# acerbilab/gpyreg

Measured on AMD Instinct MI355X. Metric: GP-fits/sec (NLL+grad, N=4096 D=10), higher is better.
Workload: dtype f64

## Files before the change

### gpyreg_amd/_lib.py

```python

from __future__ import annotations

import ctypes as C
import os
import threading

import numpy as np

_HERE = os.path.dirname(os.path.abspath(__file__))
LIB_PATH = os.environ.get("GPYREG_AMD_LIB") or os.path.join(_HERE, "lib", "libgpcore.so")

K_SE, K_MATERN, K_RQ, K_SE_ISO, K_MATERN_ISO = range(5)
F64, F32 = 0, 1
KLO_ZERO, KLO_ROW, KLO_COL = 0, 1, 2
KHI_FULL, KHI_ROW, KHI_COL = 0, 1, 2

_dp = C.c_void_p
_ip = C.c_void_p
_vp = C.c_void_p
_dpp = C.POINTER(C.c_double)

SIGNATURES = {
    "gpc_create": (C.c_int, [C.c_int, C.POINTER(_vp)]),
    "gpc_destroy": (None, [_vp]),
# ... 331 lines not shown
        self._check(self._lib.gpc_set_option(self._h, name.encode(), int(value)), "gpc_set_option")

    @_serial
    def get_option(self, name: str) -> int:
        v = C.c_int()
        self._check(self._lib.gpc_get_option(self._h, name.encode(), C.byref(v)), "gpc_get_option")
        return v.value

    @_serial
    def last_lauum_timing(self):
        a, b = C.c_double(), C.c_double()
        self._lib.gpc_last_lauum_timing(self._h, C.byref(a), C.byref(b))
        return a.value, b.value

    @_serial
    def mfma_peak(self, dtype=F64):
        t, cyc, ghz = C.c_double(), C.c_double(), C.c_double()
        rc = self._lib.gpc_mfma_peak(self._h, dtype, C.byref(t), C.byref(cyc), C.byref(ghz))
        self._check(rc, "gpc_mfma_peak")
        return t.value, cyc.value, ghz.value

    @_serial
    def debug_gemm(self, A, B, Cm, M, N, K, a_kmajor, b_kmajor, alpha=1.0, beta=0, klo=0, khi=0,
                   lower_only=False, dtype=F64, force_bt=0):
        A, B = _f64(A), _f64(B)
        Cm = _f64(Cm).copy()
        flags = int(bool(lower_only)) | {0: 0, 64: 0x100, 128: 0x200, 12864: 0x400}[force_bt]
        rc = self._lib.gpc_debug_gemm(self._h, dtype, M, N, K, int(a_kmajor), int(b_kmajor),
                                      float(alpha), int(beta), klo, khi, flags, _ptr(A),
                                      _ptr(B), _ptr(Cm))
        self._check(rc, "gpc_debug_gemm")
        return Cm

    @_serial
    def debug_factor(self, A, want_inv=True, dtype=F64):
        A = _f64(A)
        n = A.shape[0]
        L, W = np.empty((n, n)), np.empty((n, n))
        Ainv = np.empty((n, n)) if want_inv else None
        logdet = C.c_double()
        info = C.c_int()
        rc = self._lib.gpc_debug_factor(self._h, dtype, n, _ptr(A), _ptr(L), _ptr(W), _ptr(Ainv),
                                        C.byref(logdet), C.byref(info))
        self._check(rc, "gpc_debug_factor")
        return L, W, Ainv, logdet.value, info.value

    @_serial
    def debug_cov(self, which, kid, degree, hyp_cov, X, dtype=F64, kscale=1.0, sl=1.0, dvec=None, X_star=None,
                  mat=None, vec=None):
        code = {"build": 0, "front": 1, "cross": 2, "trace": 3}[which]
# ... 340 lines not shown
```

### gpyreg_amd/csrc/common.h

```cpp
#pragma once
#include <hip/hip_runtime.h>

#include <cmath>
#include <cstdint>
#include <cstdio>
#include <cstring>
#include <string>
#include <vector>

namespace gpc {

constexpr int TILE = 128;
constexpr int WAVE = 64;

inline int pad_tile(int n) { return ((n + TILE - 1) / TILE) * TILE; }

inline int chunk_from_budget(int S, size_t per, size_t shared, size_t budget, bool clamp_to_one) {
  if (budget < shared + per) return clamp_to_one ? 1 : 0;
  const size_t fit = (budget - shared) / per;
  return (int)(fit < (size_t)S ? fit : (size_t)S);
}

constexpr int LEAF_TIMEOUT = 1 << 30;

template <typename T>
struct MM;

template <>
struct MM<double> {
  using acc_t = double __attribute__((ext_vector_type(4)));
// ... 50 lines not shown
__device__ __forceinline__ bool cu_reserve_bail(const unsigned short* __restrict__ tbl, int* __restrict__ ctr) {
  __shared__ int bail_sh;
  if (threadIdx.x == 0) {
    unsigned hw, xcc;
    asm volatile("s_getreg_b32 %0, hwreg(HW_REG_HW_ID)" : "=s"(hw));
    asm volatile("s_getreg_b32 %0, hwreg(HW_REG_XCC_ID)" : "=s"(xcc));
    const unsigned cu = (hw >> 8) & 0xf, se = (hw >> 13) & 0x7;
    int bail = (tbl[(xcc & 7) * 8 + se] >> cu) & 1;
    if (!bail) {
      __hip_atomic_fetch_add(ctr + CTR_SURVIVORS, 1, __ATOMIC_RELAXED, __HIP_MEMORY_SCOPE_AGENT);
      __hip_atomic_fetch_add(ctr + CTR_STARTED, 1, __ATOMIC_RELEASE, __HIP_MEMORY_SCOPE_AGENT);
    } else {
      const int before = __hip_atomic_fetch_add(ctr + CTR_STARTED, 1, __ATOMIC_ACQ_REL, __HIP_MEMORY_SCOPE_AGENT);
      if (before == (int)gridDim.x - 1 &&
          __hip_atomic_load(ctr + CTR_SURVIVORS, __ATOMIC_ACQUIRE, __HIP_MEMORY_SCOPE_AGENT) == 0)
        bail = 0;
    }
    bail_sh = bail;
  }
  __syncthreads();
  return bail_sh != 0;
}

}
```

### gpyreg_amd/csrc/gemm.h

```cpp
#pragma once
#include "common.h"

#include <type_traits>

namespace gpc {

template <typename T>
constexpr int BKT_v = sizeof(T) == 4 ? 32 : 16;
template <typename T>
constexpr bool MM_SWZ = sizeof(T) == 4;
template <typename T>
constexpr int LDQ_v = MM_SWZ<T> ? BKT_v<T> : BKT_v<T> + 1;
constexpr int ldp_of(int BT) { return BT + 16; }
template <typename T>
constexpr int opsz_of(int BT) {
  return BKT_v<T> * (BT + 16) > BT * LDQ_v<T> ? BKT_v<T> * (BT + 16) : BT * LDQ_v<T>;
}

enum { KLO_ZERO = 0, KLO_ROW = 1, KLO_COL = 2 };
enum { KHI_FULL = 0, KHI_ROW = 1, KHI_COL = 2 };

struct GemmArgs {
  const void* A;
  const void* B;
  void* C;
  long long sA, sB, sC;
  int lda, ldb, ldc;
  int M, N, K;
  double alpha;
  int beta;
  int klo, khi, lower_only;
  int tiles_m, tiles_n;
  int flags = 0;
  const unsigned short* rsv = nullptr;
  int* ctr = nullptr;
  int ntiles = 0, batch = 0;
  double* colsq = nullptr;
  const double* ep_w = nullptr;
  long long ep_sw = 0;
  const double* ep_alpha = nullptr;
};
inline int g_gemm_flags = 8 | 16;

template <typename T, bool KM, int BT, int NT>
__device__ __forceinline__ unsigned stage_toff(int ld, int t) {
  constexpr int VEC = MM<T>::VEC;
  if constexpr (!KM) {
    constexpr int TPR = BKT_v<T> / VEC;
    return (unsigned)(t / TPR) * (unsigned)ld + (unsigned)((t % TPR) * VEC);
  } else {
    constexpr int VPR = BT / VEC;
    return (unsigned)(t / VPR) * (unsigned)ld + (unsigned)((t % VPR) * VEC);
  }
}
template <typename T, bool KM, int BT, int NT>
// ... 62 lines not shown
      return s[(r0 + l15) * LDQ_v<T> + (((k / VEC) ^ ((l15 >> 1) & 7)) * VEC) + (k % VEC)];
    } else {
      return s[(r0 + (lane & 15)) * LDQ_v<T> + kk + (lane >> 4)];
    }
  }
  else
    return s[(kk + (lane >> 4)) * ldp_of(BT) + r0 + (lane & 15)];
}

__device__ __forceinline__ void tri_tile(int tile, int& ti, int& tj) {
  int i = (int)((sqrtf(8.f * (float)tile + 1.f) - 1.f) * 0.5f);
  while (i * (i + 1) / 2 > tile) --i;
  while ((i + 1) * (i + 2) / 2 <= tile) ++i;
  ti = i;
  tj = tile - i * (i + 1) / 2;
}

#ifdef GPC_TILE_TRACE
__device__ unsigned long long g_tile_trace[2][4];
#define TILE_TS(k) do { if (HO && threadIdx.x == 0) { const long long _n = wall_clock64(); atomicAdd(&g_tile_trace[BT == 64][k], (unsigned long long)(_n - _ts)); _ts = _n; } } while (0)
#else
#define TILE_TS(k) do { } while (0)
#endif
template <typename T, bool AKM, bool BKM, int BT, int NW, int HO = 0, int EPI = 0, int BTN = BT>
__device__ __forceinline__ void gemm_tile(const GemmArgs& g, const int bx, const int by, T* __restrict__ smem) {
#ifdef GPC_TILE_TRACE
  long long _ts = wall_clock64();
  if (HO && threadIdx.x == 0) atomicAdd(&g_tile_trace[BT == 64][3], 1ull);
#endif
  using acc_t = typename MM<T>::acc_t;
  using vec_t = typename MM<T>::vec_t;
  constexpr int NT = 64 * NW;
  constexpr int NVA = (BT * BKT_v<T>) / (NT * MM<T>::VEC), NVB = (BTN * BKT_v<T>) / (NT * MM<T>::VEC);
  constexpr int OPSZA = opsz_of<T>(BT), OPSZB = opsz_of<T>(BTN), STG = OPSZA + OPSZB;
  constexpr int WCOLS = NW / 2;
  constexpr int WTM = BT / 2;
  constexpr int WTN = BTN / WCOLS;
  constexpr int MRM = WTM / 16, MRN = WTN / 16;
  static_assert(NVA >= 1 && NVB >= 1 && MRM >= 1 && MRN >= 1, "tile shape");
  const int t = threadIdx.x;
  const int lane = t & 63, w = t >> 6, wr = w / WCOLS, wc = w % WCOLS;

  int ti, tj;
  if (g.lower_only) {
    if constexpr (BTN == BT) {
      tri_tile(bx, ti, tj);
    } else {
      static_assert(BT == 2 * BTN, "lower tiles of a rectangular launch: two tile columns per tile row");
      int i = (int)((sqrtf(4.f * (float)bx + 1.f) - 1.f) * 0.5f);
      while (i * (i + 1) > bx) --i;
      while ((i + 1) * (i + 2) <= bx) ++i;
      ti = i;
      tj = bx - i * (i + 1);
    }
  } else if (g.khi == KHI_COL) {
    tj = g.tiles_n - 1 - bx / g.tiles_m;
    ti = bx % g.tiles_m;
  } else if (g.klo == KLO_COL) {
    tj = bx / g.tiles_m;
    ti = bx % g.tiles_m;
  } else if (g.khi == KHI_ROW) {
    ti = g.tiles_m - 1 - bx / g.tiles_n;
    tj = bx % g.tiles_n;
  } else {
    ti = bx / g.tiles_n;
    tj = bx % g.tiles_n;
  }
  const int m0 = ti * BT, n0 = tj * BTN;
  const int m128 = (m0 / TILE) * TILE, n128 = (n0 / TILE) * TILE;
  int k0 = g.klo == KLO_ROW ? m128 : (g.klo == KLO_COL ? n128 : 0);
  int k1 = g.khi == KHI_ROW ? m128 + TILE : (g.khi == KHI_COL ? n128 + TILE : g.K);
  if (k1 > g.K) k1 = g.K;
  const int nk = (k1 - k0) / BKT_v<T>;

  const T* __restrict__ A = reinterpret_cast<const T*>(g.A) + (size_t)by * g.sA;
  const T* __restrict__ B = reinterpret_cast<const T*>(g.B) + (size_t)by * g.sB;
  T* __restrict__ C = reinterpret_cast<T*>(g.C) + (size_t)by * g.sC;

  acc_t acc[MRM][MRN];
#pragma unroll
  for (int i = 0; i < MRM; ++i)
#pragma unroll
    for (int j = 0; j < MRN; ++j) acc[i][j] = acc_t{0, 0, 0, 0};
  constexpr bool TWO_LEVEL = sizeof(T) == 4;
  acc_t acc2[TWO_LEVEL ? MRM : 1][TWO_LEVEL ? MRN : 1];
  if constexpr (TWO_LEVEL) {
#pragma unroll
    for (int i = 0; i < MRM; ++i)
#pragma unroll
      for (int j = 0; j < MRN; ++j) acc2[i][j] = acc_t{0, 0, 0, 0};
  }

  if (nk > 0) {
    vec_t ra[NVA], rb[NVB];
    const unsigned toa = stage_toff<T, AKM, BT, NT>(g.lda, t) * (unsigned)sizeof(T),
                   tob = stage_toff<T, BKM, BTN, NT>(g.ldb, t) * (unsigned)sizeof(T);
// ... 12 lines not shown
        ua += (unsigned)(BKT_v<T> * sizeof(T));
      }
      if constexpr (BKM) {
        pb += rowsb;
        rsb = make_rsrc(pb);
      } else {
        ub += (unsigned)(BKT_v<T> * sizeof(T));
      }
    };
    constexpr int AUX = HO == 1 ? 16 : 0;
    g2r<T, AKM, BT, NT, AUX>(ra, rsa, ua, psa, toa);
    g2r<T, BKM, BTN, NT, AUX>(rb, rsb, ub, psb, tob);
    r2s<T, AKM, BT, NT>(smem, ra, t);
    r2s<T, BKM, BTN, NT>(smem + OPSZA, rb, t);
    next_slab();
    g2r<T, AKM, BT, NT, AUX>(ra, rsa, ua, psa, toa);
    g2r<T, BKM, BTN, NT, AUX>(rb, rsb, ub, psb, tob);
    __syncthreads();
    TILE_TS(0);

    T af[2][MRM], bf[2][MRN];
    auto load_frags = [&](int set, const T* a_s, const T* b_s, int kk) {
#pragma unroll
      for (int i = 0; i < MRM; ++i) af[set][i] = frag<T, AKM, BT>(a_s, wr * WTM + i * 16, kk, lane);
#pragma unroll
      for (int j = 0; j < MRN; ++j) bf[set][j] = frag<T, BKM, BTN>(b_s, wc * WTN + j * 16, kk, lane);
    };
    auto mfmas = [&](int set) {
#pragma unroll
      for (int i = 0; i < MRM; ++i)
#pragma unroll
        for (int j = 0; j < MRN; ++j) acc[i][j] = MM<T>::mma(af[set][i], bf[set][j], acc[i][j]);
    };
    constexpr int NMEM = NVA + NVB;
    constexpr int PER = (MRM * MRN) / NMEM;
    constexpr int REM = MRM * MRN - PER * NMEM;
    static_assert(PER >= 1, "interleave pattern");
    constexpr int KS = BKT_v<T> / 4;
    static_assert(KS >= 4 && KS % 2 == 0, "fragment sets alternate per k-step and wrap per slab");
    auto slab = [&](auto cur_c, auto wr_c, auto ld_c) {
      constexpr int CUR = decltype(cur_c)::value;
      constexpr bool WR = decltype(wr_c)::value, LD = decltype(ld_c)::value;
      const T* a_s = smem + CUR * STG;
      const T* b_s = a_s + OPSZA;
      T* a_n = smem + (CUR ^ 1) * STG;
#pragma unroll
      for (int ks = 0; ks < KS - 2; ++ks) {
        load_frags((ks + 1) & 1, a_s, b_s, 4 * (ks + 1));
        mfmas(ks & 1);
        __builtin_amdgcn_sched_group_barrier(0x100, MRM + MRN, 0);
        __builtin_amdgcn_sched_group_barrier(0x008, MRM * MRN, 0);
      }
      load_frags(1, a_s, b_s, 4 * (KS - 1));
      mfmas(0);
      if constexpr (WR) {
        r2s<T, AKM, BT, NT>(a_n, ra, t);
        r2s<T, BKM, BTN, NT>(a_n + OPSZA, rb, t);
      }
      __builtin_amdgcn_sched_group_barrier(0x100, MRM + MRN, 0);
#pragma unroll
      for (int q = 0; q < NMEM; ++q) {
        __builtin_amdgcn_sched_group_barrier(0x008, PER, 0);
        if constexpr (WR) __builtin_amdgcn_sched_group_barrier(0x200, 1, 0);
      }
      if constexpr (REM > 0) __builtin_amdgcn_sched_group_barrier(0x008, REM, 0);
      __syncthreads();
      if constexpr (LD) {
        next_slab();
        g2r<T, AKM, BT, NT, AUX>(ra, rsa, ua, psa, toa);
        g2r<T, BKM, BTN, NT, AUX>(rb, rsb, ub, psb, tob);
      }
      if constexpr (WR) load_frags(0, a_n, a_n + OPSZA, 0);
      mfmas(1);
      if constexpr (WR) __builtin_amdgcn_sched_group_barrier(0x100, MRM + MRN, 0);
#pragma unroll
      for (int q = 0; q < NMEM; ++q) {
        __builtin_amdgcn_sched_group_barrier(0x008, PER, 0);
        if constexpr (LD) __builtin_amdgcn_sched_group_barrier(0x020, 1, 0);
      }
      if constexpr (REM > 0) __builtin_amdgcn_sched_group_barrier(0x008, REM, 0);
    };
    using I0 = std::integral_constant<int, 0>;
    using I1 = std::integral_constant<int, 1>;
    load_frags(0, smem, smem + OPSZA, 0);
    int it = 0;
    for (; it + 3 < nk; it += 2) {
      slab(I0{}, std::true_type{}, std::true_type{});
      slab(I1{}, std::true_type{}, std::true_type{});
      if constexpr (TWO_LEVEL) {
#pragma unroll
        for (int i = 0; i < MRM; ++i)
#pragma unroll
          for (int j = 0; j < MRN; ++j) {
            acc2[i][j] += acc[i][j];
            acc[i][j] = acc_t{0, 0, 0, 0};
          }
      }
    }
    slab(I0{}, std::true_type{}, std::false_type{});
    slab(I1{}, std::false_type{}, std::false_type{});
  }

  TILE_TS(1);
// ... 69 lines not shown
    for (int j = 0; j < MRN; ++j) {
      cs[j] += __shfl_xor(cs[j], 16, 64);
      cs[j] += __shfl_xor(cs[j], 32, 64);
    }
    double* red = reinterpret_cast<double*>(smem);
    __syncthreads();
    if ((lane >> 4) == 0) {
#pragma unroll
      for (int j = 0; j < MRN; ++j) red[wr * BT + wc * WTN + j * 16 + (lane & 15)] = cs[j];
    }
    __syncthreads();
    if (t < BT) g.colsq[((size_t)by * g.tiles_m + ti) * (size_t)g.N + n0 + t] = red[t] + red[BT + t];
    __syncthreads();
    return;
  }
#pragma unroll
  for (int i = 0; i < MRM; ++i) {
    T old[MRN][4];
    if (g.beta) {
#pragma unroll
      for (int j = 0; j < MRN; ++j)
#pragma unroll
        for (int r = 0; r < 4; ++r) {
          const int row = m0 + wr * WTM + i * 16 + MM<T>::row_of(lane, r);
          const int col = n0 + wc * WTN + j * 16 + (lane & 15);
          if constexpr (HO == 1)
            old[j][r] = __hip_atomic_load(&C[(size_t)row * g.ldc + col], __ATOMIC_RELAXED, __HIP_MEMORY_SCOPE_AGENT);
          else
            old[j][r] = C[(size_t)row * g.ldc + col];
        }
    }
#pragma unroll
    for (int j = 0; j < MRN; ++j)
#pragma unroll
      for (int r = 0; r < 4; ++r) {
        const int row = m0 + wr * WTM + i * 16 + MM<T>::row_of(lane, r);
        const int col = n0 + wc * WTN + j * 16 + (lane & 15);
        T v;
        if constexpr (TWO_LEVEL)
          v = alpha * (acc[i][j][r] + acc2[i][j][r]);
        else
          v = alpha * acc[i][j][r];
        if (g.beta) v += old[j][r];
        if constexpr (HO)
          __hip_atomic_store(&C[(size_t)row * g.ldc + col], v, __ATOMIC_RELAXED, __HIP_MEMORY_SCOPE_AGENT);
        else
          C[(size_t)row * g.ldc + col] = v;
      }
  }
  TILE_TS(2);
}

template <typename T, bool AKM, bool BKM, int BT, int NW, int EPI = 0, int BTN = BT>
__global__ __launch_bounds__(64 * NW, NW / 2) void gemm_kernel(GemmArgs g) {
  __shared__ __attribute__((aligned(16))) T smem[2 * (opsz_of<T>(BT) + opsz_of<T>(BTN))];
  int bx = blockIdx.x, by = blockIdx.y;
  if ((g.flags & 16) && gridDim.y >= 8) {
    const int total = gridDim.x * gridDim.y, per = total >> 3;
    const int L = blockIdx.y * gridDim.x + blockIdx.x;
    if (L < (per << 3)) {
      const int wk = (L & 7) * per + (L >> 3);
      bx = wk % (int)gridDim.x;
      by = wk / (int)gridDim.x;
    }
  }
  gemm_tile<T, AKM, BKM, BT, NW, 0, EPI, BTN>(g, bx, by, smem);
}

template <typename T, bool A1, bool B1, bool A2, bool B2, int BT, int NW>
__global__ __launch_bounds__(64 * NW, NW / 2) void gemm_dual_kernel(GemmArgs g1, GemmArgs g2, int n1) {
  __shared__ __attribute__((aligned(16))) T smem[4 * opsz_of<T>(BT)];
  int bx = blockIdx.x, by = blockIdx.y;
  if ((g1.flags & 16) && gridDim.y >= 8) {
// ... 260 lines not shown
```

### gpyreg_amd/csrc/gpcore.hip

```cpp
#include "../../include/gpcore.h"

#include <algorithm>
#include <atomic>
#include <chrono>
#include <cmath>
#include <cstdlib>
#include <cstring>
#include <memory>
#include <mutex>

#include "blas1.h"
#include "block_append.h"
#include "common.h"
#include "covfun.h"
#include "draw.h"
#include "gemm.h"
#include "leaf.h"
#include "lookahead.h"
#include "paths.h"
#include "plan.h"
#include "quad.h"
#include "quad_mix.h"
#ifdef GPC_EXPERIMENTS
#include "dag.h"
// ... 355 lines not shown
  hipStream_t sst[MAXG + 1] = {};
  static constexpr int NDEV = 64;
  hipEvent_t dev_ev[MAXG + 1][NDEV] = {};
  hipEvent_t ev_bfork[MAXG + 1] = {}, ev_btail[MAXG + 1] = {};
  int defer_min = -1, defer_reserve = 8;
  unsigned cu_seen[64] = {};
  bool cu_map_ok = false;
  DevBuf rsv_tbl;
  int nll_block = -1;
  int solves_beside_lauum = 1;
#ifdef GPC_EXPERIMENTS
  int rl_panel = 0;
  int rl_ahead_max = 8;
#endif
  int stable = 0;
  int small_path = 1;
  int small_poll = 1, small_timing = 0;
  double* land_blk = nullptr;
  static constexpr size_t LAND_BYTES = 64u << 10;
  unsigned long long land_seq = 0;
  unsigned long long small_polled = 0, small_synced = 0;
  unsigned long long cov_fused = 0;
  unsigned long long quad_mix_gemms = 0;
  int check_queues = 0;
  hipEvent_t ev_up = nullptr, ev_done[MAXG] = {};
  int groups = 2;
  hipEvent_t ev_l0[MAXG + 1] = {}, ev_l1[MAXG + 1] = {};
  double ms_lauum = 0, flops_lauum = 0;
  int lauum_groups = 0;
  std::string err;
  std::string devinfo;
  int N = 0, D = 0, npad = 0;
  DevBuf dX;
  DevBuf dY;
  std::vector<double> hy;
  DevBuf mA, mW, mT;
  DevBuf xs, spb, mulb, divb;
  DevBuf dvec, rvec, zvec, avec;
  DevBuf tpart;
  DevBuf scal;
  DevBuf parts, gout, diagq;
  DevBuf dmb, dsn2b, mg, ng;
  DevBuf ks, vb, kss, xss, pout;
  DevBuf qb, gpart, gres;
  DevBuf qcon;
  DevBuf qmix;
// ... 447 lines not shown
                         (const double*)xs, (const double*)spb, dv, N, npad, Ac, sM, npad, ntl_head, ntl, n,
                         reserve_tbl(), bctr);
        HIPCHK(c, hipEventRecord(c->ev_btail[gidx], sd));
      } else {
        GPC_COV_DISPATCH(build_kernel, T, b.cd, dim3(ntl, n), dim3(256), 0, st, b.cd, (const double*)xs,
                         (const double*)spb, dv, N, npad, Ac, sM, npad, 0);
      }
    }
    HIPCHK(c, hipGetLastError());

    if (f0 && !c->capturing) HIPCHK(c, hipEventRecord(f0, st));
    Factor<T> F;
    F.st = st;
    F.batch = n;
    F.npad = npad;
    F.A = Ac;
    F.W = Wc;
    F.Tm = Tc;
    F.sA = F.sW = F.sT = sM;
    F.logdet = d_logdet;
    F.info = d_info;
    F.nvalid = N;
    F.stable = stable || c->stable;
    if ((defer_node > 0 || use_rl) && !c->capturing && gpc::g_persist_spare >= 0) {
      F.side = c->sst[gidx];
      F.evs = c->dev_ev[gidx];
      F.nev = gpc_ctx::NDEV - 2;
      F.defer_min = defer_node;
      F.reserve = reserve_tbl();
    }
#ifdef GPC_EXPERIMENTS
    if (indep_mode && !c->capturing) {
      F.reserve = c->rsv_tbl4.template as<unsigned short>();
      F.reserved_small_bt = 64;
      F.reserve_all = true;
      F.reserve_min = c->indep_min_tiles;
    }
#endif
    if (c->check_queues && !c->capturing) F.qlog = &qlog;
    if (split_build) {
      F.ev_tail = c->ev_btail[gidx];
      F.tail_row0 = 1024;
    }
    if (gpc::g_persist_spare >= 0) {
      F.ctr = c->tile_ctr.as<int>() + (size_t)gidx * gpc_ctx::CTR_PER_GROUP;
      F.ctr_cap = gpc_ctx::CTR_PER_GROUP - CTR_STRIDE;
// ... 61 lines not shown
                             npad, tpart, d_quad);
        else
          hipLaunchKernelGGL((trmv_t_part_kernel<T, 8>), gt, dim3(256), 0, sx, (const T*)Wc, sM, npad, (const double*)zvec,
                             npad, tpart, d_quad);
        hipLaunchKernelGGL(trmv_t_sum_kernel, dim3(npad / 128, n), dim3(128), 0, sx, (const double*)tpart, npad,
                           (const double*)spb, (int)SP_STRIDE, (int)SP_SL, avec);
      }
      HIPCHK(c, hipGetLastError());
      return 0;
    };
    hipEvent_t ev_solved = nullptr;
    if (mode == MODE_GRAD) {
      if (solves_beside_lauum) {
        hipStream_t sx = c->sst[gidx];
        hipEvent_t ev_fork = c->dev_ev[gidx][gpc_ctx::NDEV - 1];
        ev_solved = c->dev_ev[gidx][gpc_ctx::NDEV - 2];
        HIPCHK(c, hipEventRecord(ev_fork, st));
        HIPCHK(c, hipStreamWaitEvent(sx, ev_fork, 0));
        if (int rc = solves(sx)) return rc;
        HIPCHK(c, hipEventRecord(ev_solved, sx));
      }
      if (!dag_has_lauum) {
        if (!c->capturing) HIPCHK(c, hipEventRecord(c->ev_l0[gidx], st));
        F.lauum(Tc, sM);
        if (!c->capturing) {
          HIPCHK(c, hipEventRecord(c->ev_l1[gidx], st));
          lauum_n[gidx] = n;
        }
      }
    }
    HIPCHK(c, F.err);
    HIPCHK(c, hipGetLastError());
    if (f1 && !c->capturing) HIPCHK(c, hipEventRecord(f1, st));
    c->last_flops += F.flops;

    if (ev_solved)
      HIPCHK(c, hipStreamWaitEvent(st, ev_solved, 0));
    else if (int rc = solves(st))
      return rc;
    HIPCHK(c, hipGetLastError());

    const int Pn = P();
    if (mode == MODE_GRAD) {
      double* parts = c->parts.as<double>() + (size_t)off * ntl * Pn;
      double* diagq = c->diagq.as<double>() + (size_t)off * npad;
      if (kmode()) {
        hipLaunchKernelGGL((diagq_kernel<T>), dim3(1, n), dim3(256), 0, st, (const T*)Tc, sM, npad, (const double*)avec,
// ... 1934 lines not shown

template <typename T>
int debug_gemm_impl(gpc_ctx* c, int M, int N, int K, int akm, int bkm, double alpha, int beta, int klo,
                    int khi, int lower, const double* A, const double* B, double* C) {
  if (upload_as<T>(c, c->dbg1, A, (size_t)M * K)) return -1;
  if (upload_as<T>(c, c->dbg2, B, (size_t)N * K)) return -1;
  if (upload_as<T>(c, c->dbg3, C, (size_t)M * N)) return -1;
  GemmArgs g;
  g.A = c->dbg1.p;
  g.B = c->dbg2.p;
  g.C = c->dbg3.p;
  g.sA = g.sB = g.sC = 0;
  g.lda = akm ? M : K;
  g.ldb = bkm ? N : K;
  g.ldc = N;
  g.M = M;
  g.N = N;
  g.K = K;
  g.alpha = alpha;
  g.beta = beta;
  g.klo = klo;
  g.khi = khi;
  g.lower_only = lower & 1;
  g.tiles_n = N / TILE;
  HIPCHK(c, launch_gemm<T>(c->st, g, akm != 0, bkm != 0, 1, (lower & 0x100) ? 64 : ((lower & 0x200) ? 128 : ((lower & 0x400) ? 12864 : 0))));
  return download_as<T>(c, c->dbg3.as<T>(), C, (size_t)M * N);
}

template <typename T>
int debug_factor_impl(gpc_ctx* c, int n, const double* A, double* L, double* W, double* Ainv,
                      double* logdet, int* info) {
  const int npad = pad_tile(n);
  const size_t msz = (size_t)npad * npad;
  HIPCHK(c, c->mA.ensure(msz * sizeof(T)));
  HIPCHK(c, c->mW.ensure(msz * sizeof(T)));
  HIPCHK(c, c->mT.ensure(msz * sizeof(T)));
  HIPCHK(c, c->dbg1.ensure((size_t)n * n * 8));
  HIPCHK(c, c->scal.ensure(64));
  HIPCHK(c, hipMemcpyAsync(c->dbg1.p, A, (size_t)n * n * 8, hipMemcpyHostToDevice, c->st));
  HIPCHK(c, hipMemsetAsync(c->scal.p, 0, 64, c->st));
  dim3 blk(64, 4), gp(npad / 64, npad / 4);
  hipLaunchKernelGGL((pad_load_kernel<T>), gp, blk, 0, c->st, c->dbg1.as<double>(), n, npad, c->mA.as<T>());
  Factor<T> F;
  F.st = c->st;
  F.batch = 1;
  F.npad = npad;
// ... 1842 lines not shown
#ifdef GPC_EXPERIMENTS
constexpr int IS_EXPERIMENTS_BUILD = 1;
#else
constexpr int IS_EXPERIMENTS_BUILD = 0;
#endif
int clamp_to(int lo, int hi, int v) { return std::max(lo, std::min(hi, v)); }
int tile_multiple(int v) { return std::max(TILE, (v / TILE) * TILE); }
int engine_choice(int v) { return v == 1 || v == 2 ? v : 0; }
#define GPC_GET(expr) [](gpc_ctx* c) -> int { (void)c; return (int)(expr); }
#define GPC_SET(stmt) [](gpc_ctx* c, int v) -> int { (void)c; stmt; return 0; }
#define GPC_COUNTER(field) GPC_GET(c->field & 0x7fffffff), nullptr
const Option OPTIONS[] = {
    {"groups", GPC_GET(c->groups), GPC_SET(c->groups = clamp_to(1, gpc_ctx::MAXG, v))},
    {"small_blocks", GPC_GET(gpc::g_small_launch_blocks), GPC_SET(gpc::g_small_launch_blocks = v)},
    {"dual_launch", GPC_GET(gpc::g_dual_launch ? 1 : 0), GPC_SET(gpc::g_dual_launch = v != 0)},
    {"leaf", GPC_GET(gpc::g_leaf_version), GPC_SET(gpc::g_leaf_version = v == 3 ? 3 : 5)},
    {"defer_min", GPC_GET(c->defer_min), GPC_SET(c->defer_min = v)},
    {"defer_reserve", GPC_GET(c->defer_reserve), [](gpc_ctx* c, int v) -> int { return c->defer_reserve = v, build_reserve_table(c); }},
    {"leaf_fault", nullptr, GPC_SET(gpc::g_leaf_fault = v != 0)},
    {"nll_block", GPC_GET(c->nll_block), GPC_SET(c->nll_block = v < 0 ? -1 : (v == 0 ? 0 : tile_multiple(v)))},
    {"solves_beside_lauum", GPC_GET(c->solves_beside_lauum), GPC_SET(c->solves_beside_lauum = v != 0)},
    {"stable", GPC_GET(c->stable), GPC_SET(c->stable = v != 0)},
    {"small_path", GPC_GET(c->small_path), GPC_SET(c->small_path = v != 0)},
    {"check_queues", GPC_GET(c->check_queues), GPC_SET(c->check_queues = v != 0)},
    {"small_poll", GPC_GET(c->small_poll), GPC_SET(c->small_poll = v != 0)},
    {"small_timing", GPC_GET(c->small_timing), GPC_SET(c->small_timing = v != 0)},
    {"small_polled", GPC_COUNTER(small_polled)},
    {"small_synced", GPC_COUNTER(small_synced)},
    {"cov_fused", GPC_COUNTER(cov_fused)},
    {"quad_mix_gemms", GPC_COUNTER(quad_mix_gemms)},
    {"start_mult_log10", nullptr, GPC_SET(c->start_mult = std::pow(10.0, clamp_to(0, 9, v)))},
    {"append_fail_mask", nullptr, GPC_SET(c->append_fail_mask = (unsigned)v)},
    {"block_engine", GPC_GET(c->block_engine), GPC_SET(c->block_engine = engine_choice(v))},
    {"block_engine_ran", GPC_GET(c->block_engine_ran), nullptr},
    {"paths_engine", GPC_GET(c->paths_engine), GPC_SET(c->paths_engine = engine_choice(v))},
    {"paths_engine_ran", GPC_GET(c->paths_engine_ran), nullptr},
    {"paths_solve_engine", GPC_GET(c->paths_solve_engine), GPC_SET(c->paths_solve_engine = engine_choice(v))},
    {"paths_solve_engine_ran", GPC_GET(c->paths_solve_engine_ran), nullptr},
    {"block_appended", GPC_COUNTER(block_appended)},
    {"block_stale", GPC_COUNTER(block_stale)},
    {"experiments", GPC_GET(IS_EXPERIMENTS_BUILD), nullptr},
};
#ifdef GPC_EXPERIMENTS
#define GPC_INT_OPTION(name, lvalue, clamped) {name, GPC_GET(lvalue), GPC_SET(lvalue = (clamped))}
const Option EXPERIMENT_OPTIONS[] = {
    GPC_INT_OPTION("rect_min", gpc::g_rect_min_blocks, v),
// ... 274 lines not shown
```

### gpyreg_amd/csrc/leaf.h

```cpp
#pragma once
#include "common.h"

#include <type_traits>

namespace gpc {

__device__ __forceinline__ double rsq_estimate(double x) { return __builtin_amdgcn_rsq(x); }
__device__ __forceinline__ float rsq_estimate(float x) { return __builtin_amdgcn_rsqf(x); }
template <typename T>
struct RsqSteps {
  static constexpr int N = std::is_same<T, double>::value ? 6 : 3;
  T h, y, a, e;
  __device__ __forceinline__ void start(T x) {
    y = rsq_estimate(x);
    h = (T)0.5 * x;
  }
  __device__ __forceinline__ void step(int i) {
    switch (i % 3) {
      case 0: a = h * y; break;
      case 1: e = __builtin_fma(-a, y, (T)0.5); break;
      default: y = __builtin_fma(y, e, y); break;
    }
  }
};
// ... 29 lines not shown
        : "v"(dk), "v"(wk), "n"(J));
  else
    asm volatile(
        "v_mov_b64_dpp %2, %3 row_newbcast:%5 row_mask:0xf bank_mask:0xf\n\t"
        "v_fma_f64 %0, -%3, %2, %0\n\tv_fma_f64 %1, -%2, %4, %1"
        : "+v"(dj), "+v"(wj), "=&v"(t)
        : "v"(dk), "v"(wk), "n"(J));
}
template <int J, bool NOP>
__device__ __forceinline__ void elim16(float& dj, float& wj, float dk, float wk) {
  float t;
  if constexpr (NOP)
    asm volatile(
        "s_nop 1\n\tv_mov_b32_dpp %2, %3 row_newbcast:%5 row_mask:0xf bank_mask:0xf\n\t"
        "v_fma_f32 %0, -%3, %2, %0\n\tv_fma_f32 %1, -%2, %4, %1"
        : "+v"(dj), "+v"(wj), "=&v"(t)
        : "v"(dk), "v"(wk), "n"(J));
  else
    asm volatile(
        "v_mov_b32_dpp %2, %3 row_newbcast:%5 row_mask:0xf bank_mask:0xf\n\t"
        "v_fma_f32 %0, -%3, %2, %0\n\tv_fma_f32 %1, -%2, %4, %1"
        : "+v"(dj), "+v"(wj), "=&v"(t)
        : "v"(dk), "v"(wk), "n"(J));
}
template <int B, int E, typename F>
__device__ __forceinline__ void static_for(F&& f) {
  if constexpr (B < E) {
    f(std::integral_constant<int, B>{});
    static_for<B + 1, E>(f);
  }
}

template <typename T>
__device__ __forceinline__ void diag16(T (&d)[16], T (&wv)[16], int l15, int& badk) {
#pragma unroll
  for (int i = 0; i < 16; ++i) wv[i] = (l15 == i) ? (T)1 : (T)0;
  T s = bcast16<0>(d[0]);
  if (!(s > (T)0)) badk = 0;
  T r = fast_rsqrt(s);
  static_for<0, 16>([&](auto kc) {
    constexpr int k = decltype(kc)::value;
    d[k] = d[k] * r;
    wv[k] = wv[k] * r;
    __builtin_amdgcn_sched_barrier(0);
    if constexpr (k + 1 < 16) {
      elim16<k + 1, true>(d[k + 1], wv[k + 1], d[k], wv[k]);
      const T sn = bcast16<k + 1>(d[k + 1]);
      if (!(sn > (T)0) && badk < 0) badk = k + 1;
      RsqSteps<T> n;
      n.start(sn);
      __builtin_amdgcn_sched_barrier(0);
      static_for<k + 2, 16>([&](auto jc) {
        constexpr int j = decltype(jc)::value;
// ... 701 lines not shown
```

### gpyreg_amd/csrc/plan.h

```cpp
#pragma once
#include "blas1.h"
#include "gemm.h"
#include "leaf.h"

#include <algorithm>

namespace gpc {

#ifdef GPC_EXPERIMENTS
struct PlanRecorder {
  struct Op {
    int kind;
    GemmArgs g;
    bool akm, bkm;
    int off;
  };
  std::vector<Op> ops;
  bool unsupported = false;
};
#endif

template <typename T>
struct Factor {
#ifdef GPC_EXPERIMENTS
// ... 11 lines not shown
  long long sA, sW, sT;
  double* logdet;
  int* info;
  int* ctr = nullptr;
  int ctr_cap = 0, ctr_used = 0;
  hipStream_t side = nullptr;
  hipEvent_t* evs = nullptr;
  int nev = 0, ev_used = 0;
  int defer_min = 0;
  const unsigned short* reserve = nullptr;
  struct QueueCheck {
    int* slot;
    int ntiles, batch;
  };
  std::vector<QueueCheck>* qlog = nullptr;
#ifdef GPC_EXPERIMENTS
  bool reserve_all = false;
  int reserve_min = 64;
  int reserved_small_bt = 128;
#else
  static constexpr bool reserve_all = false;
  static constexpr int reserve_min = 64, reserved_small_bt = 128;
#endif
  bool dual_launch = g_dual_launch;
  bool stable = false;
  hipEvent_t ev_tail = nullptr;
  int tail_row0 = 1 << 30;
  void need_rows(int hi) {
    if (ev_tail && hi > tail_row0) {
      chk(hipStreamWaitEvent(st, ev_tail, 0));
      ev_tail = nullptr;
    }
  }
  double flops = 0;
  int launches = 0;
  hipError_t err = hipSuccess;

  T* blk(T* base, int r, int c) const { return base + (size_t)r * npad + c; }

  GemmArgs make_args(T* C, long long sC, const T* Aop, long long sAop, const T* Bop, long long sBop, int M, int N,
                     int K, double alpha, int beta, int klo, int khi, int lower) {
    GemmArgs g;
    g.A = Aop;
    g.B = Bop;
    g.C = C;
    g.sA = sAop;
    g.sB = sBop;
    g.sC = sC;
    g.lda = g.ldb = g.ldc = npad;
    g.M = M;
    g.N = N;
    g.K = K;
    g.alpha = alpha;
    g.beta = beta;
    g.klo = klo;
    g.khi = khi;
    g.lower_only = lower;
    g.tiles_n = N / TILE;
    flops += gemm_flops(g, batch);
    return g;
  }

  void gemm(T* C, long long sC, const T* Aop, long long sAop, const T* Bop, long long sBop, int M,
            int N, int K, bool akm, bool bkm, double alpha, int beta, int klo, int khi, int lower,
            hipStream_t on = nullptr, const unsigned short* rsv = nullptr) {
    GemmArgs g;
    g.A = Aop;
    g.B = Bop;
    g.C = C;
    g.sA = sAop;
    g.sB = sBop;
    g.sC = sC;
    g.lda = g.ldb = g.ldc = npad;
    g.M = M;
    g.N = N;
    g.K = K;
    g.alpha = alpha;
    g.beta = beta;
    g.klo = klo;
    g.khi = khi;
    g.lower_only = lower;
    g.tiles_n = N / TILE;
    flops += gemm_flops(g, batch);
    ++launches;
#ifdef GPC_EXPERIMENTS
    if (rec) {
      rec->ops.push_back({0, g, akm, bkm, 0});
      return;
    }
// ... 32 lines not shown
      launch_leaf<T>(st, batch, blk(A, off, off), sA, npad, blk(W, off, off), sW, npad, off, logdet, info,
                     std::max(0, std::min(TILE, nvalid - off)), stable);
      flops += (2.0 / 3.0) * TILE * (double)TILE * TILE * batch;
      ++launches;
      return;
    }
    const int q = n / TILE;
    const int n1 = (q / 2) * TILE, n2 = n - n1;
    const int o1 = off, o2 = off + n1;
    potrf_inv(o1, n1, true, keep_L);
    need_rows(o2 + n2);
    gemm(blk(Tm, o2, o1), sT, blk(A, o2, o1), sA, blk(W, o1, o1), sW, n2, n1, n1, false, false, 1.0,
         0, KLO_ZERO, KHI_COL, 0);
    if (stable) {
      gemm(blk(A, o2, o1), sA, blk(Tm, o2, o1), sT, blk(A, o1, o1), sA, n2, n1, n1, false, false, -1.0, 1, KLO_ZERO,
           KHI_COL, 0);
      gemm(blk(Tm, o2, o1), sT, blk(A, o2, o1), sA, blk(W, o1, o1), sW, n2, n1, n1, false, false, 1.0, 1, KLO_ZERO,
           KHI_COL, 0);
    }
    const bool defer = need_inv && side && defer_min > 0 && n >= defer_min && ev_used + 2 <= nev;
    bool u_done = false;
    {
      GemmArgs gs = make_args(blk(A, o2, o2), sA, blk(Tm, o2, o1), sT, blk(Tm, o2, o1), sT, n2, n2, n1, -1.0, 1,
                              KLO_ZERO, KHI_FULL, 1);
      const long long syrk_tiles = (long long)(n2 / TILE) * (n2 / TILE + 1) / 2 * batch;
      if (need_inv && !defer && dual_launch && !rec && gemm_is_small(gs, batch) && !(reserve_all && syrk_tiles >= reserve_min)) {
        GemmArgs gu = make_args(blk(A, o2, o1), sA, blk(Tm, o2, o1), sT, blk(W, o1, o1), sW, n2, n1, n1, 1.0, 0,
                                KLO_COL, KHI_FULL, 0);
        if (gemm_is_small(gu, batch)) {
          hipError_t e = launch_gemm_dual_small<T>(st, gs, gu, batch);
          if (e != hipSuccess && err == hipSuccess) err = e;
          ++launches;
          u_done = true;
        } else {
          flops -= gemm_flops(gu, batch);
        }
      }
      if (!u_done) {
        flops -= gemm_flops(gs, batch);
        gemm(blk(A, o2, o2), sA, blk(Tm, o2, o1), sT, blk(Tm, o2, o1), sT, n2, n2, n1, false, false, -1.0, 1,
             KLO_ZERO, KHI_FULL, 1);
      }
    }
    hipEvent_t ev_join = nullptr;
    if (defer) {
      hipEvent_t ev_fork = evs[ev_used++];
      ev_join = evs[ev_used++];
      chk(hipEventRecord(ev_fork, st));
      chk(hipStreamWaitEvent(side, ev_fork, 0));
      gemm(blk(A, o2, o1), sA, blk(Tm, o2, o1), sT, blk(W, o1, o1), sW, n2, n1, n1, false, true, 1.0, 0,
           KLO_COL, KHI_FULL, 0, side, reserve);
      chk(hipEventRecord(ev_join, side));
    }
    potrf_inv(o2, n2, need_inv, keep_L);
    if (need_inv) {
      if (defer)
        chk(hipStreamWaitEvent(st, ev_join, 0));
      else if (!u_done)
        gemm(blk(A, o2, o1), sA, blk(Tm, o2, o1), sT, blk(W, o1, o1), sW, n2, n1, n1, false, true, 1.0, 0,
             KLO_COL, KHI_FULL, 0);
      gemm(blk(W, o2, o1), sW, blk(W, o2, o2), sW, blk(A, o2, o1), sA, n2, n1, n2, false, true, -1.0,
           0, KLO_ZERO, KHI_ROW, 0);
    }
#ifdef GPC_EXPERIMENTS
// ... 21 lines not shown
      }
      return;
    }
    const int q = n / TILE;
    const int n1 = (q / 2) * TILE, n2 = n - n1;
    trsm_nll(r0, m, c0, n1);
    gemm(blk(A, r0, c0 + n1), sA, blk(Tm, r0, c0), sT, blk(Tm, c0 + n1, c0), sT, m, n2, n1, false, false, -1.0, 1,
         KLO_ZERO, KHI_FULL, 0);
    trsm_nll(r0, m, c0 + n1, n2);
  }

  void potrf_nll(int off, int n) {
    if (n <= nll_block || n == TILE) {
      potrf_inv(off, n, true, false);
      return;
    }
    const int q = n / TILE;
    const int n1 = (q / 2) * TILE, n2 = n - n1;
    const int o1 = off, o2 = off + n1;
    potrf_nll(o1, n1);
    need_rows(o2 + n2);
    trsm_nll(o2, n2, o1, n1);
    gemm(blk(A, o2, o2), sA, blk(Tm, o2, o1), sT, blk(Tm, o2, o1), sT, n2, n2, n1, false, false, -1.0, 1, KLO_ZERO,
         KHI_FULL, 1);
    potrf_nll(o2, n2);
  }

  void forward_solve_nll(int off, int n, double* r, double* z) {
    if (n <= nll_block || n == TILE) {
      hipLaunchKernelGGL((trmv_kernel<T>), dim3(n / 4, batch), dim3(256), 0, st, (const T*)W, sW, npad,
                         (const double*)r, npad, z, off);
      ++launches;
      return;
    }
    const int q = n / TILE;
    const int n1 = (q / 2) * TILE, n2 = n - n1;
    forward_solve_nll(off, n1, r, z);
    hipLaunchKernelGGL((gemv_sub_kernel<T>), dim3(n2 / 4, batch), dim3(256), 0, st, (const T*)Tm, sT, npad,
                       (const double*)z, r, npad, off + n1, off, n1);
    ++launches;
    forward_solve_nll(off + n1, n2, r, z);
  }

#ifdef GPC_EXPERIMENTS
  int rl_panel = 0;
  bool rl_lookahead = true;

// ... 50 lines not shown
#endif

  bool low_regs = false;
  void forward_solve(int off, int n, bool need_inv, double* r, double* z) {
    if (need_inv || n == TILE) {
      if (low_regs && off == 0 && n == npad)
        hipLaunchKernelGGL((trmv_low_kernel<T>), dim3(n / 16, batch), dim3(256), 0, st, (const T*)W, sW, npad,
                           (const double*)r, npad, z);
      else
        hipLaunchKernelGGL((trmv_kernel<T>), dim3(n / 4, batch), dim3(256), 0, st, (const T*)W, sW, npad,
                           (const double*)r, npad, z, off);
      ++launches;
      return;
    }
    const int q = n / TILE;
    const int n1 = (q / 2) * TILE, n2 = n - n1;
    forward_solve(off, n1, true, r, z);
    hipLaunchKernelGGL((gemv_sub_kernel<T>), dim3(n2 / 4, batch), dim3(256), 0, st, (const T*)Tm, sT, npad,
                       (const double*)z, r, npad, off + n1, off, n1);
    ++launches;
    forward_solve(off + n1, n2, need_inv, r, z);
  }

  void lauum(T* out, long long sOut) {
    gemm(out, sOut, W, sW, W, sW, npad, npad, npad, true, true, 1.0, 0, KLO_ROW, KHI_FULL, 1);
  }
};

}
```

Measured before the change: 845.9.

## Skip upper-triangle MFMAs and stores on diagonal tiles of lower-only SYRK/LAUUM GEMMs

Adds a diagonal-structured variant of the GEMM tile body that, for diagonal tiles of lower-triangular launches, issues MFMAs and epilogue stores only for the 16x16 sub-blocks on or below the diagonal. It switches to an interleaved wave-to-subblock mapping so the lower-triangle work stays spread across waves, and adjusts the scheduling group barriers to match the reduced MFMA count. It is enabled by default for the SYRK trailing updates in the Cholesky recursion and for the LAUUM product. Only diagonal tiles benefit, so the saving is a small fraction of the total GEMM work. The changed fragment mapping may also alter LDS access patterns and instruction scheduling for all EPI==0 tiles.

```diff
diff --git a/gpyreg_amd/_lib.py b/gpyreg_amd/_lib.py
--- a/gpyreg_amd/_lib.py
+++ b/gpyreg_amd/_lib.py
@@ -377,10 +377,11 @@
 
     @_serial
     def debug_gemm(self, A, B, Cm, M, N, K, a_kmajor, b_kmajor, alpha=1.0, beta=0, klo=0, khi=0,
-                   lower_only=False, dtype=F64, force_bt=0):
+                   lower_only=False, dtype=F64, force_bt=0, diag_lower=False):
         A, B = _f64(A), _f64(B)
         Cm = _f64(Cm).copy()
         flags = int(bool(lower_only)) | {0: 0, 64: 0x100, 128: 0x200, 12864: 0x400}[force_bt]
+        flags |= 0x1000 if diag_lower else 0
         rc = self._lib.gpc_debug_gemm(self._h, dtype, M, N, K, int(a_kmajor), int(b_kmajor),
                                       float(alpha), int(beta), klo, khi, flags, _ptr(A),
                                       _ptr(B), _ptr(Cm))
diff --git a/gpyreg_amd/csrc/common.h b/gpyreg_amd/csrc/common.h
--- a/gpyreg_amd/csrc/common.h
+++ b/gpyreg_amd/csrc/common.h
@@ -6,6 +6,7 @@
 #include <cstdio>
 #include <cstring>
 #include <string>
+#include <type_traits>
 #include <vector>
 
 namespace gpc {
@@ -102,4 +103,12 @@
   return bail_sh != 0;
 }
 
+template <int B, int E, typename F>
+__device__ __forceinline__ void static_for(F&& f) {
+  if constexpr (B < E) {
+    f(std::integral_constant<int, B>{});
+    static_for<B + 1, E>(f);
+  }
 }
+
+}
diff --git a/gpyreg_amd/csrc/gemm.h b/gpyreg_amd/csrc/gemm.h
--- a/gpyreg_amd/csrc/gemm.h
+++ b/gpyreg_amd/csrc/gemm.h
@@ -19,6 +19,7 @@
 
 enum { KLO_ZERO = 0, KLO_ROW = 1, KLO_COL = 2 };
 enum { KHI_FULL = 0, KHI_ROW = 1, KHI_COL = 2 };
+enum { GEMM_DIAG_LOWER = 1 };
 
 struct GemmArgs {
   const void* A;
@@ -31,6 +32,7 @@
   int beta;
   int klo, khi, lower_only;
   int tiles_m, tiles_n;
+  int structure = 0;
   int flags = 0;
   const unsigned short* rsv = nullptr;
   int* ctr = nullptr;
@@ -139,8 +141,9 @@
 #else
 #define TILE_TS(k) do { } while (0)
 #endif
-template <typename T, bool AKM, bool BKM, int BT, int NW, int HO = 0, int EPI = 0, int BTN = BT>
-__device__ __forceinline__ void gemm_tile(const GemmArgs& g, const int bx, const int by, T* __restrict__ smem) {
+template <typename T, bool AKM, bool BKM, int BT, int NW, int HO, int EPI, int BTN, bool DG>
+__device__ __forceinline__ void gemm_tile_body(const GemmArgs& g, const int by, const int ti, const int tj,
+                                               T* __restrict__ smem) {
 #ifdef GPC_TILE_TRACE
   long long _ts = wall_clock64();
   if (HO && threadIdx.x == 0) atomicAdd(&g_tile_trace[BT == 64][3], 1ull);
@@ -157,38 +160,17 @@
   static_assert(NVA >= 1 && NVB >= 1 && MRM >= 1 && MRN >= 1, "tile shape");
   const int t = threadIdx.x;
   const int lane = t & 63, w = t >> 6, wr = w / WCOLS, wc = w % WCOLS;
-
-  int ti, tj;
-  if (g.lower_only) {
-    if constexpr (BTN == BT) {
-      tri_tile(bx, ti, tj);
-    } else {
-      static_assert(BT == 2 * BTN, "lower tiles of a rectangular launch: two tile columns per tile row");
-      int i = (int)((sqrtf(4.f * (float)bx + 1.f) - 1.f) * 0.5f);
-      while (i * (i + 1) > bx) --i;
-      while ((i + 1) * (i + 2) <= bx) ++i;
-      ti = i;
-      tj = bx - i * (i + 1);
-    }
-  } else if (g.khi == KHI_COL) {
-    tj = g.tiles_n - 1 - bx / g.tiles_m;
-    ti = bx % g.tiles_m;
-  } else if (g.klo == KLO_COL) {
-    tj = bx / g.tiles_m;
-    ti = bx % g.tiles_m;
-  } else if (g.khi == KHI_ROW) {
-    ti = g.tiles_m - 1 - bx / g.tiles_n;
-    tj = bx % g.tiles_n;
-  } else {
-    ti = bx / g.tiles_n;
-    tj = bx % g.tiles_n;
-  }
+  constexpr bool IL = EPI == 0;
+  auto rgrp = [&](int i) { return IL ? (i * 2 + wr) * 16 : wr * WTM + i * 16; };
+  auto cgrp = [&](int j) { return IL ? (j * WCOLS + wc) * 16 : wc * WTN + j * 16; };
+
   const int m0 = ti * BT, n0 = tj * BTN;
   const int m128 = (m0 / TILE) * TILE, n128 = (n0 / TILE) * TILE;
   int k0 = g.klo == KLO_ROW ? m128 : (g.klo == KLO_COL ? n128 : 0);
   int k1 = g.khi == KHI_ROW ? m128 + TILE : (g.khi == KHI_COL ? n128 + TILE : g.K);
   if (k1 > g.K) k1 = g.K;
   const int nk = (k1 - k0) / BKT_v<T>;
+  static_assert(!DG || (EPI == 0 && HO == 0 && BTN == BT && NW == 4), "diagonal form: stored square tiles of 2 x 2 waves");
 
   const T* __restrict__ A = reinterpret_cast<const T*>(g.A) + (size_t)by * g.sA;
   const T* __restrict__ B = reinterpret_cast<const T*>(g.B) + (size_t)by * g.sB;
@@ -247,15 +229,16 @@
     T af[2][MRM], bf[2][MRN];
     auto load_frags = [&](int set, const T* a_s, const T* b_s, int kk) {
 #pragma unroll
-      for (int i = 0; i < MRM; ++i) af[set][i] = frag<T, AKM, BT>(a_s, wr * WTM + i * 16, kk, lane);
-#pragma unroll
-      for (int j = 0; j < MRN; ++j) bf[set][j] = frag<T, BKM, BTN>(b_s, wc * WTN + j * 16, kk, lane);
+      for (int i = 0; i < MRM; ++i) af[set][i] = frag<T, AKM, BT>(a_s, rgrp(i), kk, lane);
+#pragma unroll
+      for (int j = 0; j < MRN; ++j) bf[set][j] = frag<T, BKM, BTN>(b_s, cgrp(j), kk, lane);
     };
     auto mfmas = [&](int set) {
 #pragma unroll
       for (int i = 0; i < MRM; ++i)
 #pragma unroll
-        for (int j = 0; j < MRN; ++j) acc[i][j] = MM<T>::mma(af[set][i], bf[set][j], acc[i][j]);
+        for (int j = 0; j < MRN; ++j)
+          if (!DG || i >= j) acc[i][j] = MM<T>::mma(af[set][i], bf[set][j], acc[i][j]);
     };
     constexpr int NMEM = NVA + NVB;
     constexpr int PER = (MRM * MRN) / NMEM;
@@ -266,6 +249,7 @@
     auto slab = [&](auto cur_c, auto wr_c, auto ld_c) {
       constexpr int CUR = decltype(cur_c)::value;
       constexpr bool WR = decltype(wr_c)::value, LD = decltype(ld_c)::value;
+      constexpr int NM = DG ? MRM * (MRM + 1) / 2 : MRM * MRN;
       const T* a_s = smem + CUR * STG;
       const T* b_s = a_s + OPSZA;
       T* a_n = smem + (CUR ^ 1) * STG;
@@ -274,7 +258,7 @@
         load_frags((ks + 1) & 1, a_s, b_s, 4 * (ks + 1));
         mfmas(ks & 1);
         __builtin_amdgcn_sched_group_barrier(0x100, MRM + MRN, 0);
-        __builtin_amdgcn_sched_group_barrier(0x008, MRM * MRN, 0);
+        __builtin_amdgcn_sched_group_barrier(0x008, NM, 0);
       }
       load_frags(1, a_s, b_s, 4 * (KS - 1));
       mfmas(0);
@@ -283,12 +267,13 @@
         r2s<T, BKM, BTN, NT>(a_n + OPSZA, rb, t);
       }
       __builtin_amdgcn_sched_group_barrier(0x100, MRM + MRN, 0);
-#pragma unroll
-      for (int q = 0; q < NMEM; ++q) {
-        __builtin_amdgcn_sched_group_barrier(0x008, PER, 0);
+      static_for<0, NMEM>([&](auto q_c) {
+        constexpr int q = decltype(q_c)::value;
+        constexpr int CNT = DG ? ((q + 1) * NM) / NMEM - (q * NM) / NMEM : PER;
+        if constexpr (CNT > 0) __builtin_amdgcn_sched_group_barrier(0x008, CNT, 0);
         if constexpr (WR) __builtin_amdgcn_sched_group_barrier(0x200, 1, 0);
-      }
-      if constexpr (REM > 0) __builtin_amdgcn_sched_group_barrier(0x008, REM, 0);
+      });
+      if constexpr (!DG && REM > 0) __builtin_amdgcn_sched_group_barrier(0x008, REM, 0);
       __syncthreads();
       if constexpr (LD) {
         next_slab();
@@ -298,12 +283,13 @@
       if constexpr (WR) load_frags(0, a_n, a_n + OPSZA, 0);
       mfmas(1);
       if constexpr (WR) __builtin_amdgcn_sched_group_barrier(0x100, MRM + MRN, 0);
-#pragma unroll
-      for (int q = 0; q < NMEM; ++q) {
-        __builtin_amdgcn_sched_group_barrier(0x008, PER, 0);
+      static_for<0, NMEM>([&](auto q_c) {
+        constexpr int q = decltype(q_c)::value;
+        constexpr int CNT = DG ? ((q + 1) * NM) / NMEM - (q * NM) / NMEM : PER;
+        if constexpr (CNT > 0) __builtin_amdgcn_sched_group_barrier(0x008, CNT, 0);
         if constexpr (LD) __builtin_amdgcn_sched_group_barrier(0x020, 1, 0);
-      }
-      if constexpr (REM > 0) __builtin_amdgcn_sched_group_barrier(0x008, REM, 0);
+      });
+      if constexpr (!DG && REM > 0) __builtin_amdgcn_sched_group_barrier(0x008, REM, 0);
     };
     using I0 = std::integral_constant<int, 0>;
     using I1 = std::integral_constant<int, 1>;
@@ -419,8 +405,9 @@
       for (int j = 0; j < MRN; ++j)
 #pragma unroll
         for (int r = 0; r < 4; ++r) {
-          const int row = m0 + wr * WTM + i * 16 + MM<T>::row_of(lane, r);
-          const int col = n0 + wc * WTN + j * 16 + (lane & 15);
+          if (DG && i < j) continue;
+          const int row = m0 + rgrp(i) + MM<T>::row_of(lane, r);
+          const int col = n0 + cgrp(j) + (lane & 15);
           if constexpr (HO == 1)
             old[j][r] = __hip_atomic_load(&C[(size_t)row * g.ldc + col], __ATOMIC_RELAXED, __HIP_MEMORY_SCOPE_AGENT);
           else
@@ -431,8 +418,9 @@
     for (int j = 0; j < MRN; ++j)
 #pragma unroll
       for (int r = 0; r < 4; ++r) {
-        const int row = m0 + wr * WTM + i * 16 + MM<T>::row_of(lane, r);
-        const int col = n0 + wc * WTN + j * 16 + (lane & 15);
+        if (DG && i < j) continue;
+        const int row = m0 + rgrp(i) + MM<T>::row_of(lane, r);
+        const int col = n0 + cgrp(j) + (lane & 15);
         T v;
         if constexpr (TWO_LEVEL)
           v = alpha * (acc[i][j][r] + acc2[i][j][r]);
@@ -446,6 +434,42 @@
       }
   }
   TILE_TS(2);
+}
+
+template <typename T, bool AKM, bool BKM, int BT, int NW, int HO = 0, int EPI = 0, int BTN = BT>
+__device__ __forceinline__ void gemm_tile(const GemmArgs& g, const int bx, const int by, T* __restrict__ smem) {
+  int ti, tj;
+  if (g.lower_only) {
+    if constexpr (BTN == BT) {
+      tri_tile(bx, ti, tj);
+    } else {
+      static_assert(BT == 2 * BTN, "lower tiles of a rectangular launch: two tile columns per tile row");
+      int i = (int)((sqrtf(4.f * (float)bx + 1.f) - 1.f) * 0.5f);
+      while (i * (i + 1) > bx) --i;
+      while ((i + 1) * (i + 2) <= bx) ++i;
+      ti = i;
+      tj = bx - i * (i + 1);
+    }
+  } else if (g.khi == KHI_COL) {
+    tj = g.tiles_n - 1 - bx / g.tiles_m;
+    ti = bx % g.tiles_m;
+  } else if (g.klo == KLO_COL) {
+    tj = bx / g.tiles_m;
+    ti = bx % g.tiles_m;
+  } else if (g.khi == KHI_ROW) {
+    ti = g.tiles_m - 1 - bx / g.tiles_n;
+    tj = bx % g.tiles_n;
+  } else {
+    ti = bx / g.tiles_n;
+    tj = bx % g.tiles_n;
+  }
+  if constexpr (EPI == 0 && HO == 0 && BTN == BT && NW == 4) {
+    if ((g.structure & GEMM_DIAG_LOWER) && g.lower_only && ti == tj) {
+      gemm_tile_body<T, AKM, BKM, BT, NW, HO, EPI, BTN, true>(g, by, ti, tj, smem);
+      return;
+    }
+  }
+  gemm_tile_body<T, AKM, BKM, BT, NW, HO, EPI, BTN, false>(g, by, ti, tj, smem);
 }
 
 template <typename T, bool AKM, bool BKM, int BT, int NW, int EPI = 0, int BTN = BT>
diff --git a/gpyreg_amd/csrc/gpcore.hip b/gpyreg_amd/csrc/gpcore.hip
--- a/gpyreg_amd/csrc/gpcore.hip
+++ b/gpyreg_amd/csrc/gpcore.hip
@@ -401,6 +401,7 @@
   unsigned long long small_polled = 0, small_synced = 0;
   unsigned long long cov_fused = 0;
   unsigned long long quad_mix_gemms = 0;
+  int structured_gemm = 1;
   int check_queues = 0;
   hipEvent_t ev_up = nullptr, ev_done[MAXG] = {};
   int groups = 2;
@@ -894,6 +895,7 @@
     F.info = d_info;
     F.nvalid = N;
     F.stable = stable || c->stable;
+    F.structured = c->structured_gemm != 0;
     if ((defer_node > 0 || use_rl) && !c->capturing && gpc::g_persist_spare >= 0) {
       F.side = c->sst[gidx];
       F.evs = c->dev_ev[gidx];
@@ -1001,7 +1003,7 @@
       }
       if (!dag_has_lauum) {
         if (!c->capturing) HIPCHK(c, hipEventRecord(c->ev_l0[gidx], st));
-        F.lauum(Tc, sM);
+        F.lauum(Tc, sM, true);
         if (!c->capturing) {
           HIPCHK(c, hipEventRecord(c->ev_l1[gidx], st));
           lauum_n[gidx] = n;
@@ -2982,6 +2984,7 @@
   g.klo = klo;
   g.khi = khi;
   g.lower_only = lower & 1;
+  g.structure = (lower & 0x1000) ? GEMM_DIAG_LOWER : 0;
   g.tiles_n = N / TILE;
   HIPCHK(c, launch_gemm<T>(c->st, g, akm != 0, bkm != 0, 1, (lower & 0x100) ? 64 : ((lower & 0x200) ? 128 : ((lower & 0x400) ? 12864 : 0))));
   return download_as<T>(c, c->dbg3.as<T>(), C, (size_t)M * N);
@@ -4870,6 +4873,7 @@
     {"solves_beside_lauum", GPC_GET(c->solves_beside_lauum), GPC_SET(c->solves_beside_lauum = v != 0)},
     {"stable", GPC_GET(c->stable), GPC_SET(c->stable = v != 0)},
     {"small_path", GPC_GET(c->small_path), GPC_SET(c->small_path = v != 0)},
+    {"structured_gemm", GPC_GET(c->structured_gemm), GPC_SET(c->structured_gemm = v != 0)},
     {"check_queues", GPC_GET(c->check_queues), GPC_SET(c->check_queues = v != 0)},
     {"small_poll", GPC_GET(c->small_poll), GPC_SET(c->small_poll = v != 0)},
     {"small_timing", GPC_GET(c->small_timing), GPC_SET(c->small_timing = v != 0)},
diff --git a/gpyreg_amd/csrc/leaf.h b/gpyreg_amd/csrc/leaf.h
--- a/gpyreg_amd/csrc/leaf.h
+++ b/gpyreg_amd/csrc/leaf.h
@@ -75,13 +75,6 @@
         "v_fma_f32 %0, -%3, %2, %0\n\tv_fma_f32 %1, -%2, %4, %1"
         : "+v"(dj), "+v"(wj), "=&v"(t)
         : "v"(dk), "v"(wk), "n"(J));
-}
-template <int B, int E, typename F>
-__device__ __forceinline__ void static_for(F&& f) {
-  if constexpr (B < E) {
-    f(std::integral_constant<int, B>{});
-    static_for<B + 1, E>(f);
-  }
 }
 
 template <typename T>
diff --git a/gpyreg_amd/csrc/plan.h b/gpyreg_amd/csrc/plan.h
--- a/gpyreg_amd/csrc/plan.h
+++ b/gpyreg_amd/csrc/plan.h
@@ -57,6 +57,7 @@
   static constexpr bool reserve_all = false;
   static constexpr int reserve_min = 64, reserved_small_bt = 128;
 #endif
+  bool structured = false;
   bool dual_launch = g_dual_launch;
   bool stable = false;
   hipEvent_t ev_tail = nullptr;
@@ -74,8 +75,9 @@
   T* blk(T* base, int r, int c) const { return base + (size_t)r * npad + c; }
 
   GemmArgs make_args(T* C, long long sC, const T* Aop, long long sAop, const T* Bop, long long sBop, int M, int N,
-                     int K, double alpha, int beta, int klo, int khi, int lower) {
+                     int K, double alpha, int beta, int klo, int khi, int lower, int structure = 0) {
     GemmArgs g;
+    g.structure = (structured && !rec) ? structure : 0;
     g.A = Aop;
     g.B = Bop;
     g.C = C;
@@ -98,8 +100,9 @@
 
   void gemm(T* C, long long sC, const T* Aop, long long sAop, const T* Bop, long long sBop, int M,
             int N, int K, bool akm, bool bkm, double alpha, int beta, int klo, int khi, int lower,
-            hipStream_t on = nullptr, const unsigned short* rsv = nullptr) {
+            hipStream_t on = nullptr, const unsigned short* rsv = nullptr, int structure = 0) {
     GemmArgs g;
+    g.structure = (structured && !rec) ? structure : 0;
     g.A = Aop;
     g.B = Bop;
     g.C = C;
@@ -178,7 +181,7 @@
     bool u_done = false;
     {
       GemmArgs gs = make_args(blk(A, o2, o2), sA, blk(Tm, o2, o1), sT, blk(Tm, o2, o1), sT, n2, n2, n1, -1.0, 1,
-                              KLO_ZERO, KHI_FULL, 1);
+                              KLO_ZERO, KHI_FULL, 1, GEMM_DIAG_LOWER);
       const long long syrk_tiles = (long long)(n2 / TILE) * (n2 / TILE + 1) / 2 * batch;
       if (need_inv && !defer && dual_launch && !rec && gemm_is_small(gs, batch) && !(reserve_all && syrk_tiles >= reserve_min)) {
         GemmArgs gu = make_args(blk(A, o2, o1), sA, blk(Tm, o2, o1), sT, blk(W, o1, o1), sW, n2, n1, n1, 1.0, 0,
@@ -195,7 +198,7 @@
       if (!u_done) {
         flops -= gemm_flops(gs, batch);
         gemm(blk(A, o2, o2), sA, blk(Tm, o2, o1), sT, blk(Tm, o2, o1), sT, n2, n2, n1, false, false, -1.0, 1,
-             KLO_ZERO, KHI_FULL, 1);
+             KLO_ZERO, KHI_FULL, 1, nullptr, nullptr, GEMM_DIAG_LOWER);
       }
     }
     hipEvent_t ev_join = nullptr;
@@ -263,7 +266,7 @@
     need_rows(o2 + n2);
     trsm_nll(o2, n2, o1, n1);
     gemm(blk(A, o2, o2), sA, blk(Tm, o2, o1), sT, blk(Tm, o2, o1), sT, n2, n2, n1, false, false, -1.0, 1, KLO_ZERO,
-         KHI_FULL, 1);
+         KHI_FULL, 1, nullptr, nullptr, GEMM_DIAG_LOWER);
     potrf_nll(o2, n2);
   }
 
@@ -360,8 +363,9 @@
     forward_solve(off + n1, n2, need_inv, r, z);
   }
 
-  void lauum(T* out, long long sOut) {
-    gemm(out, sOut, W, sW, W, sW, npad, npad, npad, true, true, 1.0, 0, KLO_ROW, KHI_FULL, 1);
+  void lauum(T* out, long long sOut, bool diag_lower = false) {
+    gemm(out, sOut, W, sW, W, sW, npad, npad, npad, true, true, 1.0, 0, KLO_ROW, KHI_FULL, 1, nullptr, nullptr,
+         diag_lower ? GEMM_DIAG_LOWER : 0);
   }
 };
 
```

After: 845.8. No clear change (-0.0%).
